# AIflowerQ/InvPref_KDD_2022

Hardware: AMD Instinct MI355X
Metric: training interactions/sec, Yahoo-implicit InvPref (higher is better)
Workload: dtype f32; 1 GPU; yahoo_r3_implicit_shaped; users=15400, items=1000, envs=4, factor_num=64, scaling=strong, interactions_total=250154, global_batch=8192, interactions_per_gpu=250154, batch_per_gpu=8192, estep_every_steps=155, parallelism=single GPU

## Files before the change

invpref_kdd_2022_amd/csrc/canon_math.hpp:

```cpp
#pragma once
#include <hip/hip_runtime.h>

namespace invpref {

__device__ __forceinline__ float bits_to_float(unsigned u) { return __builtin_bit_cast(float, u); }
__device__ __forceinline__ unsigned float_to_bits(float f) { return __builtin_bit_cast(unsigned, f); }

__device__ __forceinline__ float pow2i(int n) { return bits_to_float((unsigned)(n + 127) << 23); }

__device__ __forceinline__ float c_exp(float x) {
    float n = __builtin_rintf(x * 1.44269504f);
    float r = __builtin_fmaf(n, -0.693359375f, x);
    r = __builtin_fmaf(n, 2.12194440e-4f, r);
    float p = 1.9875691500e-4f;
    p = __builtin_fmaf(p, r, 1.3981999507e-3f);
    p = __builtin_fmaf(p, r, 8.3334519073e-3f);
    p = __builtin_fmaf(p, r, 4.1665795894e-2f);
    p = __builtin_fmaf(p, r, 1.6666665459e-1f);
    p = __builtin_fmaf(p, r, 5.0000001201e-1f);
    float r2 = r * r;
    float y = __builtin_fmaf(p, r2, r);
    y = y + 1.0f;
    int ni = (int)n;
    int h = ni >> 1;
// ... 28 lines not shown
    float r = m + y;
    r = __builtin_fmaf(fe, 0.693359375f, r);
    r = (x == __builtin_inff()) ? x : r;
    r = (x == 0.0f) ? -__builtin_inff() : r;
    r = (x < 0.0f) ? __builtin_nanf("") : r;
    r = (x != x) ? x : r;
    return r;
}

__device__ __forceinline__ float c_log1p(float x) {
    float u = 1.0f + x;
    float r = c_log(u) * (x / (u - 1.0f));
    return (u == 1.0f) ? x : r;
}

__device__ __forceinline__ float c_sigmoid(float x) { return 1.0f / (1.0f + c_exp(-x)); }

__device__ __forceinline__ float c_bce(float s, float y) {
    float a = c_log1p(-s);
    a = a > -100.0f ? a : -100.0f;
    float b = c_log(s);
    b = b > -100.0f ? b : -100.0f;
    return (y - 1.0f) * a - y * b;
}

__device__ __forceinline__ float c_bce_binary(float s, float y) {
    const float x = -s, u = 1.0f + x;
    const bool one = y == 1.0f;
    float l = c_log(one ? s : u);
    const float l1p = (u == 1.0f) ? x : l * (x / (u - 1.0f));
    l = one ? l : l1p;
    l = l > -100.0f ? l : -100.0f;
    return -l;
}

__device__ __forceinline__ float c_dbce(float s, float y) {
    float d = (1.0f - s) * s;
    d = d > 1e-12f ? d : 1e-12f;
    return (s - y) / d;
}

__device__ __forceinline__ float c_sign(float x) { return (float)((x > 0.0f) - (x < 0.0f)); }

__device__ __forceinline__ float f_rcp(float x) { return __builtin_amdgcn_rcpf(x); }
__device__ __forceinline__ float f_exp(float x) { return __builtin_amdgcn_exp2f(x * 1.44269504f); }
__device__ __forceinline__ float f_log(float x) { return __builtin_amdgcn_logf(x) * 0.693147181f; }
__device__ __forceinline__ float f_sigmoid(float x) { return f_rcp(1.0f + f_exp(-x)); }
__device__ __forceinline__ float f_bce(float s, float y) {
    float a = f_log(1.0f - s);
    a = a > -100.0f ? a : -100.0f;
    float b = f_log(s);
    b = b > -100.0f ? b : -100.0f;
    return (y - 1.0f) * a - y * b;
}
__device__ __forceinline__ float f_bce_binary(float s, float y) {
    float l = f_log(y == 1.0f ? s : 1.0f - s);
    l = l > -100.0f ? l : -100.0f;
    return -l;
}
__device__ __forceinline__ float f_dbce(float s, float y) {
    float d = (1.0f - s) * s;
    d = d > 1e-12f ? d : 1e-12f;
    return (s - y) * f_rcp(d);
}

template <int CTRL>
__device__ __forceinline__ float dpp_move(float v) {
    return __builtin_bit_cast(float, __builtin_amdgcn_update_dpp(0, __builtin_bit_cast(int, v), CTRL, 0xF, 0xF, true));
}
__device__ __forceinline__ float row16_sum(float x) {
    x = x + dpp_move<0xB1>(x);
    x = x + dpp_move<0x4E>(x);
    x = x + dpp_move<0x141>(x);
    x = x + dpp_move<0x140>(x);
    return x;
}
__device__ __forceinline__ float row16_min(float x) {
    x = __builtin_fminf(x, dpp_move<0xB1>(x));
    x = __builtin_fminf(x, dpp_move<0x4E>(x));
    x = __builtin_fminf(x, dpp_move<0x141>(x));
    x = __builtin_fminf(x, dpp_move<0x140>(x));
    return x;
}
__device__ __forceinline__ float row16_max(float x) {
    x = __builtin_fmaxf(x, dpp_move<0xB1>(x));
    x = __builtin_fmaxf(x, dpp_move<0x4E>(x));
    x = __builtin_fmaxf(x, dpp_move<0x141>(x));
    x = __builtin_fmaxf(x, dpp_move<0x140>(x));
    return x;
}

}
```

invpref_kdd_2022_amd/csrc/invpref_kernels.hip:

```cpp
#include "adam_apply.hpp"
#include "launch.hpp"

using namespace invpref;

namespace {

template <int NC, bool VEC, int EMAX>
__global__ __launch_bounds__(256) void forward_kernel(DevTables t, const int64_t *__restrict__ users,
                                                      const int64_t *__restrict__ items,
                                                      const int64_t *__restrict__ envs, int64_t B, uint32_t flags,
                                                      float *__restrict__ inv, float *__restrict__ envaware,
                                                      float *__restrict__ envout) {
    extern __shared__ __attribute__((aligned(16))) float lds[];
    constexpr int DP = NC * 64;
    float *sEv = lds, *sW = lds + t.E * DP, *sb = sW + t.E * DP;
    stage_table(sEv, t.Ev, t.E, t.D, DP);
    stage_table(sW, t.W, t.E, t.D, DP);
    for (int i = threadIdx.x; i < t.E; i += blockDim.x) sb[i] = t.b[i];
    __syncthreads();
    const int l16 = threadIdx.x & 15;
    const int64_t rows_per_block = blockDim.x / kRow;
    const bool implicit = flags & INVPREF_IMPLICIT;
    for (int64_t s = blockIdx.x * rows_per_block + (threadIdx.x >> 4); s < B; s += gridDim.x * rows_per_block) {
        const int64_t u = users[s], v = items[s];
// ... 422 lines not shown
                                                          int sched_slot) {
    if (sched_state) a = sched_last_launch(sched_state, sched_table, sched_n, sched_slot);
    const int64_t total = r.end4[r.n - 1];
    for (int64_t j = blockIdx.x * (int64_t)blockDim.x + threadIdx.x; j < total; j += (int64_t)gridDim.x * blockDim.x) {
        int q = 0;
        while (j >= r.end4[q]) q++;
        const int64_t i = r.off4[q] + (j - (q ? r.end4[q - 1] : 0));
        adam_f4_at(p, g, m, v, i, a, zero_grad);
    }
}

constexpr int kEpsTableMaxE = 7;
struct EpsBase { float v[INVPREF_MAX_ENVS]; };
struct Factorials { unsigned long long f[INVPREF_MAX_ENVS + 1]; };
__device__ __forceinline__ unsigned long long unrank_packed(unsigned long long r, int E, const Factorials &fac) {
    unsigned avail = (1u << E) - 1u;
    unsigned long long out = 0;
#pragma unroll
    for (int pos = 0; pos < INVPREF_MAX_ENVS; pos++) {
        if (pos < E) {
            unsigned long long f = 1;
#pragma unroll
            for (int k = 0; k < INVPREF_MAX_ENVS; k++) f = (k == E - 1 - pos) ? fac.f[k] : f;
            const unsigned d = (unsigned)(r / f);
            r -= (unsigned long long)d * f;
            unsigned seen = 0, pick = 0;
#pragma unroll
            for (int b = 0; b < INVPREF_MAX_ENVS; b++) {
                const bool on = (avail >> b) & 1u;
                pick = (on && seen == d) ? (unsigned)b : pick;
                seen += on ? 1u : 0u;
            }
            avail &= ~(1u << pick);
            out |= (unsigned long long)pick << (4 * pos);
        }
    }
    return out;
}
__device__ __forceinline__ unsigned unrank_packed_small(unsigned r, int E) {
    unsigned c[8];
    c[0] = 0;
#pragma unroll
    for (int k = 1; k < 8; k++) { c[k] = r % (unsigned)(k + 1); r /= (unsigned)(k + 1); }
    unsigned avail = (1u << E) - 1u, out = 0;
#pragma unroll
    for (int pos = 0; pos < kEpsTableMaxE; pos++) {
        if (pos < E) {
            unsigned d = 0;
#pragma unroll
            for (int k = 0; k < 8; k++) d = (k == E - 1 - pos) ? c[k] : d;
            unsigned seen = 0, pick = 0;
#pragma unroll
            for (int b = 0; b < 8; b++) {
                const bool on = (avail >> b) & 1u;
                pick = (on && seen == d) ? (unsigned)b : pick;
                seen += on ? 1u : 0u;
            }
            avail &= ~(1u << pick);
            out |= pick << (4 * pos);
        }
    }
    return out;
}
template <typename IT>
__global__ __launch_bounds__(256) void eps_unrank_kernel(const IT *__restrict__ idx, int64_t N, int E, Factorials fac,
                                                         unsigned long long *__restrict__ packed) {
    for (int64_t s = blockIdx.x * (int64_t)blockDim.x + threadIdx.x; s < N; s += (int64_t)gridDim.x * blockDim.x)
        packed[s] = unrank_packed(min((unsigned long long)idx[s], fac.f[E] - 1ull), E, fac);
}
constexpr int kTicketShards = 32;
struct EstepFin {
    int *state;
    int64_t *ring;
    int ring_cap;
    int64_t *counts;
    int64_t *diff;
    float *class_w;
    const unsigned *perm_table;
};
__device__ __forceinline__ int ld_sc1_i(const int *p) { return __hip_atomic_load(p, __ATOMIC_RELAXED, __HIP_MEMORY_SCOPE_AGENT); }
__device__ __forceinline__ void st_sc1_i(int *p, int v) { __hip_atomic_store(p, v, __ATOMIC_RELAXED, __HIP_MEMORY_SCOPE_AGENT); }

constexpr int kEstepNumSgpr = 80;
template <int NC, bool VEC, bool NARROW>
__global__ __launch_bounds__(256) __attribute__((amdgpu_num_sgpr(kEstepNumSgpr))) void estep_assign_kernel(DevTables t, const int64_t *__restrict__ users,
                                                           const int64_t *__restrict__ items,
                                                           const float *__restrict__ scores, int64_t N, uint32_t flags,
                                                           const float *__restrict__ eps_rows,
                                                           const unsigned long long *__restrict__ eps_packed, EpsBase eps_base,
                                                           const void *__restrict__ eps_index, int eps_index_bytes,
                                                           int eps_rows_n, Factorials fac,
                                                           const int64_t *old_envs, int64_t *new_envs,
                                                           int *slabs, EstepFin fin) {
    extern __shared__ __attribute__((aligned(16))) float lds[];
    constexpr int DP = NC * 64;
    float *sEv = lds;
    int *cnt = reinterpret_cast<int *>(lds + t.E * DP);
    float *sbase = lds + t.E * DP + INVPREF_MAX_ENVS + 1;
    stage_table(sEv, t.Ev, t.E, t.D, DP);
    for (int i = threadIdx.x; i <= t.E; i += blockDim.x) cnt[i] = 0;
    unsigned *stab = reinterpret_cast<unsigned *>(sbase + INVPREF_MAX_ENVS);
    if (eps_packed || eps_index) {
#pragma unroll
        for (int k = 0; k < INVPREF_MAX_ENVS; k++)
            if (threadIdx.x == k) sbase[k] = eps_base.v[k];
    }
    const int64_t rows_per_block = blockDim.x / kRow;
    const int64_t chunk = ((N + gridDim.x - 1) / gridDim.x + rows_per_block - 1) / rows_per_block * rows_per_block;
    const int64_t s_begin = blockIdx.x * chunk, s_end = min(N, s_begin + chunk);
    auto load_idx = [&](int64_t sx) -> unsigned {
        return eps_index_bytes == 1 ? (unsigned)reinterpret_cast<const uint8_t *>(eps_index)[sx]
                                    : (unsigned)reinterpret_cast<const int32_t *>(eps_index)[sx];
    };
    if (eps_index) {
        if (fin.perm_table)
            for (int i = threadIdx.x; i < eps_rows_n; i += blockDim.x) stab[i] = fin.perm_table[i];
        else
            for (int i = threadIdx.x; i < eps_rows_n; i += blockDim.x) stab[i] = unrank_packed_small((unsigned)i, t.E);
    }
    __syncthreads();
    const int l16 = threadIdx.x & 15;
    const bool implicit = flags & INVPREF_IMPLICIT;
    float eps_thr = 0.f;
    if (eps_packed || eps_index) {
        float mx = 0.f;
#pragma unroll
        for (int k = 0; k < INVPREF_MAX_ENVS; k++) mx = (k < t.E) ? __builtin_fmaxf(mx, __builtin_fabsf(eps_base.v[k])) : mx;
        eps_thr = mx * 67108864.f * 1.001f;
    }
    const int64_t s_first = s_begin + (threadIdx.x >> 4);
    const bool idx_bulk = eps_index && eps_index_bytes == 1;
    const int lane64 = threadIdx.x & 63, grp_w = lane64 >> 4;
    auto load_bulk = [&](int blk) -> unsigned {
        const int64_t sx = s_begin + ((threadIdx.x >> 6) * 4 + (lane64 & 3)) + rows_per_block * ((int64_t)blk * 16 + (lane64 >> 2));
        return sx < s_end ? (unsigned)reinterpret_cast<const uint8_t *>(eps_index)[sx] : 0u;
    };
    unsigned bulk_cur = idx_bulk ? load_bulk(0) : 0u, bulk_next = 0u;
    unsigned idx_cur = (eps_index && !idx_bulk && s_first < s_end) ? load_idx(s_first) : 0u;
    int pass = 0;
    for (int64_t s = s_first; s < s_end; s += rows_per_block, pass++) {
        unsigned idx_next = 0u;
        if (idx_bulk) {
            const int pk = __builtin_amdgcn_readfirstlane(pass);
            if ((pk & 15) == 0) {
                if (pk) bulk_cur = bulk_next;
                bulk_next = load_bulk((pk >> 4) + 1);
            }
            const int src = (pk & 15) * 4;
            const unsigned i0 = __builtin_amdgcn_readlane(bulk_cur, src), i1 = __builtin_amdgcn_readlane(bulk_cur, src + 1);
            const unsigned i2 = __builtin_amdgcn_readlane(bulk_cur, src + 2), i3 = __builtin_amdgcn_readlane(bulk_cur, src + 3);
            idx_cur = grp_w == 0 ? i0 : (grp_w == 1 ? i1 : (grp_w == 2 ? i2 : i3));
        } else if (eps_index && s + rows_per_block < s_end) {
            idx_next = load_idx(s + rows_per_block);
        }
        const int64_t u = users[s], v = items[s];
        const float y = scores[s];
        float4 pu[NC], qi[NC], pa[NC], qa[NC];
        if (NARROW) {
            const unsigned uo = (unsigned)u * (unsigned)t.D, vo = (unsigned)v * (unsigned)t.D;
            load_row<NC, VEC>(t.Pu + uo, 0, t.D, l16, pu);
            load_row<NC, VEC>(t.Qi + vo, 0, t.D, l16, qi);
            load_row<NC, VEC>(t.Pa + uo, 0, t.D, l16, pa);
            load_row<NC, VEC>(t.Qa + vo, 0, t.D, l16, qa);
        } else {
            load_row<NC, VEC>(t.Pu, u, t.D, l16, pu);
            load_row<NC, VEC>(t.Qi, v, t.D, l16, qi);
            load_row<NC, VEC>(t.Pa, u, t.D, l16, pa);
            load_row<NC, VEC>(t.Qa, v, t.D, l16, qa);
        }
        const float p = dot2<NC>(pu, qi);
        const float sp = implicit ? c_sigmoid(p) : p;
        float qmine = 0.f;
        for (int c = 0; c < t.E; c++) {
            float4 ev[NC];
            lds_row<NC>(sEv, c, l16, ev);
            const float q = dot3<NC>(pa, qa, ev);
            qmine = (l16 == c) ? q : qmine;
        }
        float dist;
        if (implicit) {
            const float sv = sp * c_sigmoid(qmine);
            const bool binary = __builtin_amdgcn_ballot_w64(!(y == 0.0f || y == 1.0f)) == 0;
            dist = binary ? c_bce_binary(sv, y) : c_bce(sv, y);
        } else { const float r = (p + qmine) - y; dist = r * r; }
        if (eps_rows && l16 < t.E) dist = dist + eps_rows[s * t.E + l16];
        if (eps_packed || eps_index) {
            const bool need = row16_min(l16 < t.E ? dist : __builtin_inff()) < eps_thr;
            if (need) {
                if (eps_packed && l16 < t.E) dist = dist + sbase[(eps_packed[s] >> (4 * l16)) & 15ull];
                if (eps_index && l16 < t.E)
                    dist = dist + sbase[(stab[min(idx_cur, (unsigned)(eps_rows_n - 1))] >> (4 * l16)) & 15u];
            }
        }
        dist = l16 < t.E ? dist : __builtin_inff();
        const float dmin = row16_min(dist);
        const int bi_num = (int)row16_min(dist == dmin ? (float)l16 : 99.f);
        const int bi_nan = (int)row16_min(dist != dist ? (float)l16 : 99.f);
        const int bi = bi_nan < 99 ? bi_nan : bi_num;
        if (l16 == 0) {
            const int64_t was = old_envs ? old_envs[s] : (int64_t)bi;
            const bool changed = was != (int64_t)bi;
            new_envs[s] = bi;
            atomicAdd(cnt + bi, 1);
            if (changed) atomicAdd(cnt + t.E, 1);
        }
        if (!idx_bulk) idx_cur = idx_next;
    }
    __syncthreads();
    if (!fin.state) {
        for (int i = threadIdx.x; i <= t.E; i += blockDim.x) slabs[(int64_t)blockIdx.x * (t.E + 1) + i] = cnt[i];
        return;
    }
    __shared__ int s_last;
    __shared__ long long s_tot[INVPREF_MAX_ENVS + 1];
    if (threadIdx.x < 64) {
        if ((int)threadIdx.x <= t.E) {
            const int S0 = min(kTicketShards, (int)gridDim.x);
            __hip_atomic_fetch_add(fin.state + 32 + 32 * ((int)blockIdx.x % S0) + 1 + (int)threadIdx.x, cnt[threadIdx.x], __ATOMIC_RELAXED,
                                   __HIP_MEMORY_SCOPE_AGENT);
        }
        asm volatile("s_waitcnt vmcnt(0)" ::: "memory");
        if (threadIdx.x == 0) {
            const int S = min(kTicketShards, (int)gridDim.x), sh = (int)blockIdx.x % S;
            const int members = ((int)gridDim.x - sh + S - 1) / S;
            int *tk = fin.state + 32 + 32 * sh;
            int last = 0;
            if (__hip_atomic_fetch_add(tk, 1, __ATOMIC_RELAXED, __HIP_MEMORY_SCOPE_AGENT) == members - 1) {
                st_sc1_i(tk, 0);
                last = __hip_atomic_fetch_add(fin.state, 1, __ATOMIC_RELAXED, __HIP_MEMORY_SCOPE_AGENT) == S - 1;
            }
            s_last = last;
        }
    }
    for (int i = threadIdx.x; i <= t.E; i += blockDim.x) s_tot[i] = 0;
    __syncthreads();
    if (!s_last) return;
    {
        const int E1 = t.E + 1, nsl = (int)gridDim.x;
        const int S0 = min(kTicketShards, nsl);
        for (int i = threadIdx.x; i < S0 * E1; i += blockDim.x) {
            int *w = fin.state + 32 + 32 * (i / E1) + 1 + i % E1;
            const int x = ld_sc1_i(w);
            st_sc1_i(w, 0);
            atomicAdd((unsigned long long *)&s_tot[i % E1], (unsigned long long)(long long)x);
        }
        __syncthreads();
        int64_t *row = nullptr;
        if (fin.ring) row = fin.ring + (int64_t)((unsigned)fin.state[1] % (unsigned)fin.ring_cap) * E1;
        if ((int)threadIdx.x < t.E) {
            const long long c = s_tot[threadIdx.x];
            const long long r = (c + 1 < N - 1) ? c + 1 : N - 1;
            if (fin.counts) fin.counts[threadIdx.x] = c;
            if (fin.class_w) fin.class_w[threadIdx.x] = (float)((double)r / (double)N);
            if (row) row[threadIdx.x] = c;
        }
        if (threadIdx.x == 0) {
            if (fin.diff) *fin.diff = s_tot[t.E];
            if (row) row[t.E] = s_tot[t.E];
        }
        __syncthreads();
        if (threadIdx.x == 0) {
            if (fin.ring) fin.state[1] = fin.state[1] + 1;
            st_sc1_i(fin.state, 0);
        }
    }
}

__global__ __launch_bounds__(256) void env_hist_kernel(const int64_t *__restrict__ envs, int64_t N, int E,
                                                       int *__restrict__ slabs) {
    __shared__ int cnt[INVPREF_MAX_ENVS + 1];
    for (int i = threadIdx.x; i <= E; i += blockDim.x) cnt[i] = 0;
    __syncthreads();
    for (int64_t s = blockIdx.x * (int64_t)blockDim.x + threadIdx.x; s < N; s += (int64_t)gridDim.x * blockDim.x)
        atomicAdd(cnt + (int)envs[s], 1);
    __syncthreads();
    for (int i = threadIdx.x; i <= E; i += blockDim.x) slabs[(int64_t)blockIdx.x * (E + 1) + i] = cnt[i];
}

__global__ __launch_bounds__(256) void stat_envs_kernel(const int64_t *__restrict__ envs, int64_t N, int E,
                                                        const int *__restrict__ slabs, int nslabs,
                                                        int64_t *__restrict__ counts, int64_t *__restrict__ diff,
                                                        float *__restrict__ class_w, float *__restrict__ sample_w) {
    __shared__ long long tot[INVPREF_MAX_ENVS + 1];
    __shared__ float cw[INVPREF_MAX_ENVS];
    for (int i = threadIdx.x; i <= E; i += blockDim.x) tot[i] = 0;
    __syncthreads();
    long long acc[INVPREF_MAX_ENVS + 1];
#pragma unroll
    for (int c = 0; c <= INVPREF_MAX_ENVS; c++) acc[c] = 0;
// ... 82 lines not shown
#pragma unroll
    for (int c = 0; c < DC; c++)
#pragma unroll
        for (int s = 0; s < 16; s++) a[c][s] = pu[64 * c + 4 * s];
    const int tiles = (I + 15) / 16;
    const int t0 = (int)blockIdx.y * steps_per, t1 = min(tiles, t0 + steps_per);
    if (t0 >= t1) return;
    constexpr int F4 = D / 4, PER = 16 * F4 / 256;
    static_assert(PER == DC, "staging: DC float4 per thread");
    int src_off[PER], dst_off[PER], rr[PER];
#pragma unroll
    for (int j = 0; j < PER; j++) {
        const int f = threadIdx.x + 256 * j;
        rr[j] = f / F4;
        src_off[j] = 4 * (f - rr[j] * F4);
        dst_off[j] = rr[j] * RS + src_off[j];
    }
    float4 st[PER];
#pragma unroll
    for (int j = 0; j < PER; j++)
        st[j] = *reinterpret_cast<const float4 *>(Qi + (int64_t)min(t0 * 16 + rr[j], I - 1) * D + src_off[j]);
#pragma unroll
    for (int j = 0; j < PER; j++) *reinterpret_cast<float4 *>(lds + dst_off[j]) = st[j];
    __syncthreads();
    for (int t = t0; t < t1; t++) {
        const int buf = (t - t0) & 1;
        const int tn = min(t + 1, t1 - 1);
#pragma unroll
        for (int j = 0; j < PER; j++)
            st[j] = *reinterpret_cast<const float4 *>(Qi + (int64_t)min(tn * 16 + rr[j], I - 1) * D + src_off[j]);
        const float *bt = lds + buf * TILE + m * RS + k;
        f32x4_t acc[16];
#pragma unroll
        for (int s = 0; s < 16; s++) acc[s] = f32x4_t{0.f, 0.f, 0.f, 0.f};
#pragma unroll
        for (int c = 0; c < DC; c++)
#pragma unroll
            for (int s = 0; s < 16; s++)
                acc[s] = __builtin_amdgcn_mfma_f32_16x16x4f32(a[c][s], bt[64 * c + 4 * s], acc[s], 0, 0, 0);
#pragma unroll
        for (int s = 0; s < 16; s += 2) acc[s] = acc[s] + acc[s + 1];
#pragma unroll
        for (int s = 0; s < 16; s += 4) acc[s] = acc[s] + acc[s + 2];
#pragma unroll
        for (int s = 0; s < 16; s += 8) acc[s] = acc[s] + acc[s + 4];
        acc[0] = acc[0] + acc[8];
        const int item = t * 16 + m;
#pragma unroll
        for (int r = 0; r < 4; r++) {
            float p = acc[0][r];
            if (apply_sigmoid) p = c_sigmoid(p);
            const int64_t row = (int64_t)blockIdx.x * 64 + wave * 16 + 4 * k + r;
            if (row < n && item < I) out[row * (int64_t)I + item] = p;
        }
#pragma unroll
        for (int j = 0; j < PER; j++) *reinterpret_cast<float4 *>(lds + (buf ^ 1) * TILE + dst_off[j]) = st[j];
        __syncthreads();
    }
}

__global__ __launch_bounds__(256) void sample_weights_kernel(const int64_t *__restrict__ envs, int64_t N_local,
                                                             const int64_t *__restrict__ counts, int64_t N_total, int E,
                                                             float *__restrict__ class_w, float *__restrict__ sample_w) {
    __shared__ float cw[INVPREF_MAX_ENVS];
    if (threadIdx.x < E) {
        const long long c = counts[threadIdx.x];
        const long long r = (c + 1 < N_total - 1) ? c + 1 : N_total - 1;
        const float w = (float)((double)r / (double)N_total);
        cw[threadIdx.x] = w;
        if (blockIdx.x == 0 && class_w) class_w[threadIdx.x] = w;
    }
    __syncthreads();
    if (sample_w)
        for (int64_t s = blockIdx.x * (int64_t)blockDim.x + threadIdx.x; s < N_local; s += (int64_t)gridDim.x * blockDim.x)
            sample_w[s] = cw[(int)envs[s]];
}

constexpr int kMstepThreads = 512, kMstepMaxBlocks = 512;
constexpr int kEstepThreads = 256, kEstepMaxBlocks = 2048;
inline int mstep_blocks(int64_t B) {
    int64_t nb = (B + (kMstepThreads / kRow) - 1) / (kMstepThreads / kRow);
    return (int)(nb < 1 ? 1 : (nb > kMstepMaxBlocks ? kMstepMaxBlocks : nb));
}
inline int estep_blocks(int64_t N) {
    int64_t nb = (N + (kEstepThreads / kRow) - 1) / (kEstepThreads / kRow);
    static const int cap_env = std::getenv("INVPREF_ESTEP_BLOCKS") ? atoi(std::getenv("INVPREF_ESTEP_BLOCKS")) : 0;
    const int cap = cap_env > 0 && cap_env < kEstepMaxBlocks ? cap_env : kEstepMaxBlocks;
    return (int)(nb < 1 ? 1 : (nb > cap ? cap : nb));
}

template <typename F>
int with_nv(int nc, bool vec, F &&f) {
    return with_bool(vec, [&](auto vec_c) {
        return with_int<1, 2, 4>(nc, [&](auto nc_c) {
            if constexpr (!decltype(vec_c)::value && decltype(nc_c)::value != 4) return (int)INVPREF_EUNSUPPORTED;
            else return f(nc_c, vec_c);
        });
    });
}
template <typename F>
int with_nve(int nc, bool vec, int emax, F &&f) {
    return with_nv(nc, vec, [&](auto nc_c, auto vec_c) {
        return with_int<4, 8, 16>(emax, [&](auto emax_c) { return f(nc_c, vec_c, emax_c); });
    });
}

}

template <bool UNPACK, bool VEC>
__global__ __launch_bounds__(256) void pack_rows_kernel(float *__restrict__ flat, const int64_t *__restrict__ row_offsets,
                                                        int64_t n_rows, int32_t D, int64_t tail_offset, int64_t tail_len,
                                                        float *__restrict__ packed) {
    constexpr int W = VEC ? 4 : 1;
    const int64_t per_row = D / W, body = n_rows * per_row, total = body + (tail_len + W - 1) / W;
    for (int64_t i = (int64_t)blockIdx.x * blockDim.x + threadIdx.x; i < total; i += (int64_t)gridDim.x * blockDim.x) {
        float *f, *q;
        int cnt = W;
        if (i < body) {
            const int64_t r = i / per_row, c = i - r * per_row;
            f = flat + row_offsets[r] + c * W;
            q = packed + r * (int64_t)D + c * W;
        } else {
            const int64_t c = (i - body) * W;
            f = flat + tail_offset + c;
            q = packed + n_rows * (int64_t)D + c;
            if (tail_len - c < W) cnt = (int)(tail_len - c);
        }
        if (VEC && cnt == 4) {
            if (UNPACK) *reinterpret_cast<float4 *>(f) = *reinterpret_cast<const float4 *>(q);
            else *reinterpret_cast<float4 *>(q) = *reinterpret_cast<const float4 *>(f);
        } else {
            for (int k = 0; k < cnt; k++) {
                if (UNPACK) f[k] = q[k];
                else q[k] = f[k];
            }
        }
    }
}

static int pack_rows_launch(bool unpack, float *flat, const int64_t *row_offsets, int64_t n_rows, int32_t D,
                            int64_t tail_offset, int64_t tail_len, float *packed, int vec_ok, void *stream) {
    if (!flat || !packed || n_rows < 0 || D < 1 || tail_len < 0 || tail_offset < 0 || (n_rows > 0 && !row_offsets))
        return INVPREF_EINVAL;
    if (n_rows == 0 && tail_len == 0) return 0;
    const uintptr_t af = reinterpret_cast<uintptr_t>(flat), aq = reinterpret_cast<uintptr_t>(packed);
    const bool vec = vec_ok && D % 4 == 0 && tail_offset % 4 == 0 && ((af | aq) & 15u) == 0;
    const int64_t items = n_rows * (D / (vec ? 4 : 1)) + (tail_len + (vec ? 3 : 0)) / (vec ? 4 : 1);
    int64_t nb = (items + 255) / 256;
    nb = nb < 1 ? 1 : (nb > 4096 ? 4096 : nb);
    return with_bool(unpack, [&](auto unpack_c) {
        return with_bool(vec, [&](auto vec_c) {
            hipLaunchKernelGGL((pack_rows_kernel<decltype(unpack_c)::value, decltype(vec_c)::value>), dim3((unsigned)nb), dim3(256),
                               0, (hipStream_t)stream, flat, row_offsets, n_rows, D, tail_offset, tail_len, packed);
            return (int)hipGetLastError();
        });
    });
}

template <bool BACKWARD>
static int launch_mstep_atomic(const InvPrefTables *tables, const InvPrefTables *grads, const int64_t *users,
                               const int64_t *items, const int64_t *envs, const float *scores, const float *sample_weights,
                               int64_t B, const StepScalars &k, uint32_t flags, const Upstream &up, float l2, float l1,
                               int64_t batch_norm, float *losses6, void *workspace, hipStream_t st) {
    const DevTables t = dev_tables(tables);
    const DevGrads g = dev_grads(grads);
    const bool vec = vec_ok(tables) && vec_ok(grads);
    const int nc = vec ? nc_of(t.D) : 4, emax = emax_of(t.E);
    const int DP = nc * 64, EDP = t.E * DP;
// ... 183 lines not shown
         reinterpret_cast<uintptr_t>(exp_avg_sq)) & 15u)
        return INVPREF_EINVAL;
    if (sched && (!sched->state || !sched->table || sched->n <= 0)) return INVPREF_EINVAL;
    AdamRanges r{};
    int64_t total = 0;
    for (int i = 0; i < n_ranges; i++) {
        if (offsets[i] < 0 || lengths[i] <= 0 || (offsets[i] & 3) || (lengths[i] & 3)) return INVPREF_EINVAL;
        r.off4[i] = offsets[i] >> 2;
        total += lengths[i] >> 2;
        r.end4[i] = total;
    }
    r.n = n_ranges;
    int64_t nb = (total + 255) / 256;
    if (nb > 2048) nb = 2048;
    hipLaunchKernelGGL(adam_ranges_kernel, dim3((unsigned)nb), dim3(256), 0, (hipStream_t)stream, param, grad, exp_avg,
                       exp_avg_sq, r, a, zero_grad, sched ? sched->state : nullptr,
                       sched ? reinterpret_cast<const SchedRow *>(sched->table) : nullptr, sched ? sched->n : 0,
                       sched ? (sched->slot & 1) : 0);
    return (int)hipGetLastError();
}

int invpref_adam_ranges_hip(float *param, float *grad, float *exp_avg, float *exp_avg_sq, const int64_t *offsets,
                            const int64_t *lengths, int32_t n_ranges, int64_t step, double lr, double beta1, double beta2,
                            double eps, int zero_grad, void *stream) {
    if (step < 1) return INVPREF_EINVAL;
    return adam_ranges_launch(param, grad, exp_avg, exp_avg_sq, offsets, lengths, n_ranges,
                              adam_scalars(step, lr, beta1, beta2, eps), zero_grad, nullptr, stream);
}

int invpref_adam_ranges_sched_hip(float *param, float *grad, float *exp_avg, float *exp_avg_sq, const int64_t *offsets,
                                  const int64_t *lengths, int32_t n_ranges, const InvPrefAdamSchedule *sched,
                                  int zero_grad, void *stream) {
    if (!sched) return INVPREF_EINVAL;
    return adam_ranges_launch(param, grad, exp_avg, exp_avg_sq, offsets, lengths, n_ranges, AdamScalars{}, zero_grad,
                              sched, stream);
}

size_t invpref_estep_workspace_bytes(const InvPrefTables *tables, int64_t N) {
    const int64_t E = tables ? tables->env_num : INVPREF_MAX_ENVS;
    return sizeof(int) * (size_t)(E + 1) * kEstepMaxBlocks + sizeof(unsigned long long) * (size_t)(N > 0 ? N : 0);
}

int invpref_stat_envs_hip(const int64_t *envs, int64_t N, int64_t env_num, int64_t *counts, float *class_weights,
                          float *sample_weights, void *workspace, size_t workspace_bytes, void *stream) {
    if (!envs || !counts || !workspace || N <= 0 || env_num <= 0) return INVPREF_EINVAL;
    if (env_num > INVPREF_MAX_ENVS) return INVPREF_EUNSUPPORTED;
    if (workspace_bytes < sizeof(int) * (size_t)(env_num + 1) * kEstepMaxBlocks) return INVPREF_EWORKSPACE;
    int64_t nb = (N + 255) / 256;
    if (nb > kEstepMaxBlocks) nb = kEstepMaxBlocks;
    hipStream_t st = (hipStream_t)stream;
    int *slabs = (int *)workspace;
    hipLaunchKernelGGL(env_hist_kernel, dim3((unsigned)nb), dim3(256), 0, st, envs, N, (int)env_num, slabs);
    hipLaunchKernelGGL(stat_envs_kernel, dim3((unsigned)nb), dim3(256), 0, st, envs, N, (int)env_num, slabs, (int)nb,
                       counts, (int64_t *)nullptr, class_weights, sample_weights);
    return (int)hipGetLastError();
}

int invpref_sample_weights_hip(const int64_t *envs, int64_t N_local, const int64_t *counts, int64_t N_total,
                               int64_t env_num, float *class_weights, float *sample_weights, void *stream) {
    if (!counts || N_local < 0 || N_total <= 0 || env_num <= 0 || (N_local > 0 && sample_weights && !envs))
        return INVPREF_EINVAL;
    if (env_num > INVPREF_MAX_ENVS) return INVPREF_EUNSUPPORTED;
    int64_t nb = (N_local + 255) / 256;
    if (nb < 1) nb = 1;
    if (nb > kEstepMaxBlocks) nb = kEstepMaxBlocks;
    hipLaunchKernelGGL(sample_weights_kernel, dim3((unsigned)nb), dim3(256), 0, (hipStream_t)stream, envs, N_local, counts,
                       N_total, (int)env_num, class_weights, sample_weights);
    return (int)hipGetLastError();
}

static int estep_launch(const InvPrefTables *tables, const int64_t *users, const int64_t *items, const float *scores,
                        int64_t N, uint32_t flags, const float *eps_rows, const void *perm_index, int index_bytes,
                        const float *eps_base_host, const int64_t *old_envs, int64_t *new_envs, int64_t *counts,
                        int64_t *diff, float *class_weights, float *sample_weights, void *workspace,
                        size_t workspace_bytes, void *stream, const EstepFin *fused = nullptr) {
    int rc = check_tables(tables);
    if (rc) return rc;
    if (N <= 0 || !users || !items || !scores || !new_envs || !workspace) return INVPREF_EINVAL;
    if (!fused && (!counts || !diff)) return INVPREF_EINVAL;
    if (workspace_bytes < invpref_estep_workspace_bytes(tables, N)) return INVPREF_EWORKSPACE;
    const DevTables t = dev_tables(tables);
    const bool vec = vec_ok(tables);
    const int nc = vec ? nc_of(t.D) : 4;
    const int nb = estep_blocks(N);
    const size_t lds = sizeof(float) * ((size_t)t.E * nc * 64 + INVPREF_MAX_ENVS + 1 + INVPREF_MAX_ENVS);
    hipStream_t st = (hipStream_t)stream;
    int *slabs = (int *)workspace;
    unsigned long long *eps_packed = nullptr;
    EpsBase eps_base{};
    Factorials fac{};
    fac.f[0] = 1;
    for (int k = 1; k <= INVPREF_MAX_ENVS; k++) fac.f[k] = fac.f[k - 1] * (unsigned long long)k;
    const void *eps_index = nullptr;
    int eps_rows_n = 0;
    size_t lds_extra = 0;
    if (perm_index) {
        if (eps_rows || !eps_base_host || (index_bytes != 1 && index_bytes != 4 && index_bytes != 8)) return INVPREF_EINVAL;
        if ((index_bytes == 1 && t.E > 5) || (index_bytes == 4 && t.E > 12)) return INVPREF_EINVAL;
        for (int k = 0; k < t.E; k++) eps_base.v[k] = eps_base_host[k];
    }
    bool table_form = perm_index && t.E <= kEpsTableMaxE && index_bytes != 8;
    if (table_form) {
        lds_extra = sizeof(unsigned) * (size_t)fac.f[t.E];
        if (lds + lds_extra > 64 * 1024) { table_form = false; lds_extra = 0; }
    }
    if (table_form) {
        eps_index = perm_index;
        eps_rows_n = (int)fac.f[t.E];
    } else if (perm_index) {
        eps_packed = reinterpret_cast<unsigned long long *>(reinterpret_cast<char *>(workspace) +
                                                           sizeof(int) * (size_t)(t.E + 1) * kEstepMaxBlocks);
        int64_t ub = (N + 255) / 256;
        if (ub > 4096) ub = 4096;
        with_int<1, 4, 8>(index_bytes, [&](auto bytes_c) {
            constexpr int W = decltype(bytes_c)::value;
            using IT = std::conditional_t<W == 1, uint8_t, std::conditional_t<W == 4, int32_t, int64_t>>;
            hipLaunchKernelGGL(eps_unrank_kernel<IT>, dim3((unsigned)ub), dim3(256), 0, st, (const IT *)perm_index, N, t.E, fac,
                               eps_packed);
            return 0;
        });
    }
    EstepFin fin{};
    if (fused) {
        fin = *fused;
        if (!table_form) fin.perm_table = nullptr;
    }
    static const bool force64 = std::getenv("INVPREF_ESTEP_OFFSETS64") != nullptr && std::getenv("INVPREF_ESTEP_OFFSETS64")[0] == '1';
    const bool narrow = !force64 && (uint64_t)std::max(t.U, t.I) * (uint64_t)t.D * 4u < (1ull << 32);
    rc = with_nv(nc, vec, [&](auto nc_c, auto vec_c) {
        return with_bool(narrow, [&](auto narrow_c) {
            hipLaunchKernelGGL((estep_assign_kernel<decltype(nc_c)::value, decltype(vec_c)::value, decltype(narrow_c)::value>),
                               dim3(nb), dim3(kEstepThreads), lds + lds_extra, st, t, users, items, scores, N, flags, eps_rows,
                               eps_packed, eps_base, eps_index, index_bytes, eps_rows_n, fac, old_envs, new_envs, slabs, fin);
            return (int)hipGetLastError();
        });
    });
    if (rc) return rc;
    if (fused) return 0;
    int64_t nb2 = (N + 255) / 256;
    if (nb2 > 256) nb2 = 256;
    hipLaunchKernelGGL(stat_envs_kernel, dim3((unsigned)nb2), dim3(256), 0, st, new_envs, N, t.E, slabs, nb, counts, diff,
                       class_weights, sample_weights);
    return (int)hipGetLastError();
}

int invpref_estep_hip(const InvPrefTables *tables, const int64_t *users, const int64_t *items, const float *scores,
                      int64_t N, uint32_t flags, const float *eps_rows, const int64_t *old_envs, int64_t *new_envs,
                      int64_t *counts, int64_t *diff, float *class_weights, float *sample_weights, void *workspace,
                      size_t workspace_bytes, void *stream) {
    return estep_launch(tables, users, items, scores, N, flags, eps_rows, nullptr, 0, nullptr, old_envs, new_envs, counts,
                        diff, class_weights, sample_weights, workspace, workspace_bytes, stream);
}

int invpref_estep_perm_hip(const InvPrefTables *tables, const int64_t *users, const int64_t *items, const float *scores,
                           int64_t N, uint32_t flags, const void *perm_index, int index_bytes, const float *eps_base,
                           const int64_t *old_envs, int64_t *new_envs, int64_t *counts, int64_t *diff,
                           float *class_weights, float *sample_weights, void *workspace, size_t workspace_bytes,
                           void *stream) {
    if (!perm_index) return INVPREF_EINVAL;
    return estep_launch(tables, users, items, scores, N, flags, nullptr, perm_index, index_bytes, eps_base, old_envs,
                        new_envs, counts, diff, class_weights, sample_weights, workspace, workspace_bytes, stream);
}

int invpref_perm_table_fill(int32_t env_num, uint32_t *host_table) {
    if (!host_table || env_num < 1 || env_num > kEpsTableMaxE) return INVPREF_EINVAL;
    int rows = 1;
    for (int k = 2; k <= env_num; k++) rows *= k;
    for (int r = 0; r < rows; r++) {
        unsigned avail = (1u << env_num) - 1u, out = 0;
        int rem = r, f = rows;
        for (int pos = 0; pos < env_num; pos++) {
            f /= (env_num - pos);
            const int d = rem / f;
            rem -= d * f;
            int seen = 0, pick = 0;
            for (int b = 0; b < env_num; b++)
                if ((avail >> b) & 1u) { if (seen == d) pick = b; seen++; }
            avail &= ~(1u << pick);
            out |= (unsigned)pick << (4 * pos);
        }
        host_table[r] = out;
    }
    return rows;
}

int invpref_estep_fused_hip(const InvPrefTables *tables, const int64_t *users, const int64_t *items, const float *scores,
                            int64_t N, uint32_t flags, const void *perm_index, int index_bytes, const float *eps_base,
                            const uint32_t *perm_table, int64_t *envs, int32_t *state, int64_t *ring, int32_t ring_cap,
                            int64_t *counts, int64_t *diff, float *class_weights, void *workspace, size_t workspace_bytes,
                            void *stream) {
    if (!state || !envs || (ring && ring_cap <= 0)) return INVPREF_EINVAL;
    EstepFin fin{};
    fin.state = state; fin.ring = ring; fin.ring_cap = ring_cap; fin.counts = counts; fin.diff = diff;
    fin.class_w = class_weights; fin.perm_table = perm_table;
    return estep_launch(tables, users, items, scores, N, flags, nullptr, perm_index, perm_index ? index_bytes : 0, eps_base, envs,
                        envs, counts, diff, class_weights, nullptr, workspace, workspace_bytes, stream, &fin);
}

}
```

Before: 533.6 million interactions/s.

## Pack four samples per 16-lane group in E-step assign with DPP env lanes

Adds a packed E-step variant for D<=64 and E<=4. Each 16-lane row group processes four samples, fetching IDs through DPP quad broadcasts. Each lane of a quad then owns one environment's distance, with argmin done by quad DPP reductions. This cuts the rows-per-pass redundancy and per-sample overhead, launches more rows per block, and requests high occupancy via waves_per_eu. It adds branching complexity and register pressure and only runs when the shape constraints hold.

```diff
diff --git a/invpref_kdd_2022_amd/csrc/canon_math.hpp b/invpref_kdd_2022_amd/csrc/canon_math.hpp
--- a/invpref_kdd_2022_amd/csrc/canon_math.hpp
+++ b/invpref_kdd_2022_amd/csrc/canon_math.hpp
@@ -134,6 +134,20 @@
     x = __builtin_fminf(x, dpp_move<0x140>(x));
     return x;
 }
+__device__ __forceinline__ float quad_min(float x) {
+    x = __builtin_fminf(x, dpp_move<0xB1>(x));
+    x = __builtin_fminf(x, dpp_move<0x4E>(x));
+    return x;
+}
+template <int J>
+__device__ __forceinline__ unsigned quad_bcast(unsigned v) {
+    return (unsigned)__builtin_amdgcn_update_dpp(0, (int)v, J * 0x55, 0xF, 0xF, true);
+}
+template <int J>
+__device__ __forceinline__ float quad_keep(float old, float v) {
+    return __builtin_bit_cast(float, __builtin_amdgcn_update_dpp(__builtin_bit_cast(int, old), __builtin_bit_cast(int, v), 0xE4, 0xF,
+                                                                 1 << J, false));
+}
 __device__ __forceinline__ float row16_max(float x) {
     x = __builtin_fmaxf(x, dpp_move<0xB1>(x));
     x = __builtin_fmaxf(x, dpp_move<0x4E>(x));
diff --git a/invpref_kdd_2022_amd/csrc/invpref_kernels.hip b/invpref_kdd_2022_amd/csrc/invpref_kernels.hip
--- a/invpref_kdd_2022_amd/csrc/invpref_kernels.hip
+++ b/invpref_kdd_2022_amd/csrc/invpref_kernels.hip
@@ -528,8 +528,9 @@
 __device__ __forceinline__ void st_sc1_i(int *p, int v) { __hip_atomic_store(p, v, __ATOMIC_RELAXED, __HIP_MEMORY_SCOPE_AGENT); }
 
 constexpr int kEstepNumSgpr = 80;
-template <int NC, bool VEC, bool NARROW>
-__global__ __launch_bounds__(256) __attribute__((amdgpu_num_sgpr(kEstepNumSgpr))) void estep_assign_kernel(DevTables t, const int64_t *__restrict__ users,
+constexpr int kEstepPackedMaxE = 4;
+template <int NC, bool VEC, bool NARROW, bool PACKED>
+__global__ __launch_bounds__(256) __attribute__((amdgpu_num_sgpr(kEstepNumSgpr), amdgpu_waves_per_eu(PACKED ? 8 : 1))) void estep_assign_kernel(DevTables t, const int64_t *__restrict__ users,
                                                            const int64_t *__restrict__ items,
                                                            const float *__restrict__ scores, int64_t N, uint32_t flags,
                                                            const float *__restrict__ eps_rows,
@@ -551,7 +552,7 @@
         for (int k = 0; k < INVPREF_MAX_ENVS; k++)
             if (threadIdx.x == k) sbase[k] = eps_base.v[k];
     }
-    const int64_t rows_per_block = blockDim.x / kRow;
+    const int64_t rows_per_block = PACKED ? blockDim.x / 4 : blockDim.x / kRow;
     const int64_t chunk = ((N + gridDim.x - 1) / gridDim.x + rows_per_block - 1) / rows_per_block * rows_per_block;
     const int64_t s_begin = blockIdx.x * chunk, s_end = min(N, s_begin + chunk);
     auto load_idx = [&](int64_t sx) -> unsigned {
@@ -574,6 +575,129 @@
         for (int k = 0; k < INVPREF_MAX_ENVS; k++) mx = (k < t.E) ? __builtin_fmaxf(mx, __builtin_fabsf(eps_base.v[k])) : mx;
         eps_thr = mx * 67108864.f * 1.001f;
     }
+    if constexpr (PACKED) {
+        static_assert(NC == 1 && VEC, "the packed loop is written for one float4 chunk per lane");
+        const int wave = __builtin_amdgcn_readfirstlane((int)(threadIdx.x >> 6));
+        const unsigned lane64 = threadIdx.x & 63u, e4 = l16 & 3;
+        const unsigned off_g = (lane64 >> 4) * 4 + e4, off_c = lane64 >> 2;
+        const unsigned off_b = (lane64 >> 4) * (unsigned)rows_per_block + (lane64 & 15u);
+        const bool row_on = l16 * 4 < t.D;
+        const unsigned lane_byte = row_on ? (unsigned)l16 * 16u : 0u;
+        const unsigned row_bytes = (unsigned)t.D * 4u;
+        const int64_t w_first = s_begin + wave * 16;
+        auto room = [&](int64_t base, int cap) -> unsigned {
+            const int64_t r = s_end - 1 - base;
+            return (unsigned)__builtin_amdgcn_readfirstlane((int)(r < cap ? r : cap));
+        };
+        auto at = [](auto *arr, int64_t base, unsigned byte_off) -> auto & {
+            using T = std::remove_pointer_t<decltype(arr)>;
+            using C = std::conditional_t<std::is_const_v<T>, const char, char>;
+            auto *p = arr + base;
+            asm("" : "+s"(p));
+            return *reinterpret_cast<T *>(reinterpret_cast<C *>(p) + byte_off);
+        };
+        const bool idx_bulk = eps_index && eps_index_bytes == 1;
+        auto load_bulk = [&](int64_t base) -> unsigned {
+            const unsigned lim = room(base, 255);
+            return off_b <= lim ? (unsigned)at(reinterpret_cast<const uint8_t *>(eps_index), base, off_b) : 0u;
+        };
+        auto load_ids = [&](int64_t base, unsigned &ur, unsigned &vr, float &y, unsigned &idx) {
+            const unsigned lim = room(base, 15), og = min(off_g, lim), oc = min(off_c, lim);
+            const int64_t u = at(users, base, og * 8u), v = at(items, base, og * 8u);
+            if constexpr (NARROW) { ur = (unsigned)u * row_bytes; vr = (unsigned)v * row_bytes; }
+            else { ur = (unsigned)u; vr = (unsigned)v; }
+            const float yy = at(scores, base, oc * 4u);
+            y = off_c <= lim ? yy : 0.f;
+            if (eps_index && !idx_bulk) idx = (unsigned)at(reinterpret_cast<const int32_t *>(eps_index), base, oc * 4u);
+        };
+        auto row = [&](const float *tab, unsigned r) -> float4 {
+            const char *b = reinterpret_cast<const char *>(tab);
+            if constexpr (NARROW) return *reinterpret_cast<const float4 *>(b + (r + lane_byte));
+            else {
+                uint64_t off = (uint64_t)r * row_bytes + lane_byte;
+                asm("" : "+v"(off));
+                return *reinterpret_cast<const float4 *>(b + off);
+            }
+        };
+        unsigned ur_n = 0, vr_n = 0;
+        float y_n = 0.f;
+        unsigned idx_n = 0u, bulk_cur = 0u, bulk_next = 0u;
+        if (w_first < s_end) {
+            load_ids(w_first, ur_n, vr_n, y_n, idx_n);
+            if (idx_bulk) bulk_next = load_bulk(w_first);
+        }
+        int pass = 0;
+        for (int64_t base = w_first; base < s_end; base += rows_per_block, pass++) {
+            const unsigned ur = ur_n, vr = vr_n;
+            const float y = y_n;
+            unsigned idx_cur = idx_n;
+            const unsigned lim = room(base, 15);
+            if (base + rows_per_block < s_end) load_ids(base + rows_per_block, ur_n, vr_n, y_n, idx_n);
+            if (idx_bulk) {
+                if ((pass & 3) == 0) {
+                    bulk_cur = bulk_next;
+                    bulk_next = base + 4 * rows_per_block < s_end ? load_bulk(base + 4 * rows_per_block) : 0u;
+                }
+                idx_cur = (unsigned)__builtin_amdgcn_ds_bpermute((int)(((pass & 3) * 16 + off_c) * 4), (int)bulk_cur);
+            }
+            float pq = 0.f, qc[kEstepPackedMaxE] = {0.f, 0.f, 0.f, 0.f};
+            auto inner = [&](auto jc) {
+                constexpr int J = decltype(jc)::value;
+                const unsigned uj = quad_bcast<J>(ur), vj = quad_bcast<J>(vr);
+                const float4 pu = row(t.Pu, uj), qi = row(t.Qi, vj), pa = row(t.Pa, uj), qa = row(t.Qa, vj);
+                float sp = 0.f;
+                sp = __builtin_fmaf(pu.x, qi.x, sp); sp = __builtin_fmaf(pu.y, qi.y, sp);
+                sp = __builtin_fmaf(pu.z, qi.z, sp); sp = __builtin_fmaf(pu.w, qi.w, sp);
+                pq = quad_keep<J>(pq, row16_sum(row_on ? sp : 0.f));
+                const float4 ab = f4mul(pa, qa);
+#pragma unroll
+                for (int c = 0; c < kEstepPackedMaxE; c++) {
+                    float4 ev[1];
+                    lds_row<1>(sEv, min(c, t.E - 1), l16, ev);
+                    float sq = 0.f;
+                    sq = __builtin_fmaf(ab.x, ev[0].x, sq); sq = __builtin_fmaf(ab.y, ev[0].y, sq);
+                    sq = __builtin_fmaf(ab.z, ev[0].z, sq); sq = __builtin_fmaf(ab.w, ev[0].w, sq);
+                    qc[c] = quad_keep<J>(qc[c], row16_sum(row_on ? sq : 0.f));
+                }
+            };
+            inner(std::integral_constant<int, 0>{});
+            asm volatile("" ::: "memory");
+            inner(std::integral_constant<int, 1>{});
+            asm volatile("" ::: "memory");
+            inner(std::integral_constant<int, 2>{});
+            asm volatile("" ::: "memory");
+            inner(std::integral_constant<int, 3>{});
+            asm volatile("" ::: "memory");
+            const float qmine = e4 == 0 ? qc[0] : (e4 == 1 ? qc[1] : (e4 == 2 ? qc[2] : qc[3]));
+            const bool live = off_c <= lim, lane_on = live && (int)e4 < t.E;
+            float dist;
+            if (implicit) {
+                const float sv = c_sigmoid(pq) * c_sigmoid(qmine);
+                const bool binary = __builtin_amdgcn_ballot_w64(!(y == 0.0f || y == 1.0f)) == 0;
+                dist = binary ? c_bce_binary(sv, y) : c_bce(sv, y);
+            } else { const float r = (pq + qmine) - y; dist = r * r; }
+            if (eps_rows && lane_on) dist = dist + at(eps_rows, base * t.E, (off_c * (unsigned)t.E + e4) * 4u);
+            if (eps_packed || eps_index) {
+                const bool need = quad_min(lane_on ? dist : __builtin_inff()) < eps_thr;
+                if (need && lane_on) {
+                    if (eps_packed) dist = dist + sbase[(at(eps_packed, base, off_c * 8u) >> (4 * e4)) & 15ull];
+                    if (eps_index) dist = dist + sbase[(stab[min(idx_cur, (unsigned)(eps_rows_n - 1))] >> (4 * e4)) & 15u];
+                }
+            }
+            dist = lane_on ? dist : __builtin_inff();
+            const float dmin = quad_min(dist);
+            const int bi_num = (int)quad_min(dist == dmin ? (float)e4 : 99.f);
+            const int bi_nan = (int)quad_min(dist != dist ? (float)e4 : 99.f);
+            const int bi = bi_nan < 99 ? bi_nan : bi_num;
+            if (e4 == 0 && live) {
+                const int64_t was = old_envs ? at(old_envs, base, off_c * 8u) : (int64_t)bi;
+                const bool changed = was != (int64_t)bi;
+                at(new_envs, base, off_c * 8u) = bi;
+                atomicAdd(cnt + bi, 1);
+                if (changed) atomicAdd(cnt + t.E, 1);
+            }
+        }
+    } else {
     const int64_t s_first = s_begin + (threadIdx.x >> 4);
     const bool idx_bulk = eps_index && eps_index_bytes == 1;
     const int lane64 = threadIdx.x & 63, grp_w = lane64 >> 4;
@@ -651,6 +775,7 @@
             if (changed) atomicAdd(cnt + t.E, 1);
         }
         if (!idx_bulk) idx_cur = idx_next;
+    }
     }
     __syncthreads();
     if (!fin.state) {
@@ -899,8 +1024,8 @@
     int64_t nb = (B + (kMstepThreads / kRow) - 1) / (kMstepThreads / kRow);
     return (int)(nb < 1 ? 1 : (nb > kMstepMaxBlocks ? kMstepMaxBlocks : nb));
 }
-inline int estep_blocks(int64_t N) {
-    int64_t nb = (N + (kEstepThreads / kRow) - 1) / (kEstepThreads / kRow);
+inline int estep_blocks(int64_t N, int per_pass = kEstepThreads / kRow) {
+    int64_t nb = (N + per_pass - 1) / per_pass;
     static const int cap_env = std::getenv("INVPREF_ESTEP_BLOCKS") ? atoi(std::getenv("INVPREF_ESTEP_BLOCKS")) : 0;
     const int cap = cap_env > 0 && cap_env < kEstepMaxBlocks ? cap_env : kEstepMaxBlocks;
     return (int)(nb < 1 ? 1 : (nb > cap ? cap : nb));
@@ -1250,7 +1375,8 @@
     const DevTables t = dev_tables(tables);
     const bool vec = vec_ok(tables);
     const int nc = vec ? nc_of(t.D) : 4;
-    const int nb = estep_blocks(N);
+    const bool packed = nc == 1 && t.E <= kEstepPackedMaxE;
+    const int nb = packed ? estep_blocks(N, kEstepThreads / 4) : estep_blocks(N);
     const size_t lds = sizeof(float) * ((size_t)t.E * nc * 64 + INVPREF_MAX_ENVS + 1 + INVPREF_MAX_ENVS);
     hipStream_t st = (hipStream_t)stream;
     int *slabs = (int *)workspace;
@@ -1297,10 +1423,16 @@
     const bool narrow = !force64 && (uint64_t)std::max(t.U, t.I) * (uint64_t)t.D * 4u < (1ull << 32);
     rc = with_nv(nc, vec, [&](auto nc_c, auto vec_c) {
         return with_bool(narrow, [&](auto narrow_c) {
-            hipLaunchKernelGGL((estep_assign_kernel<decltype(nc_c)::value, decltype(vec_c)::value, decltype(narrow_c)::value>),
-                               dim3(nb), dim3(kEstepThreads), lds + lds_extra, st, t, users, items, scores, N, flags, eps_rows,
-                               eps_packed, eps_base, eps_index, index_bytes, eps_rows_n, fac, old_envs, new_envs, slabs, fin);
-            return (int)hipGetLastError();
+            return with_bool(packed, [&](auto packed_c) {
+                constexpr int NC = decltype(nc_c)::value;
+                if constexpr (decltype(packed_c)::value && NC != 1) return (int)INVPREF_EUNSUPPORTED;
+                else {
+                    hipLaunchKernelGGL((estep_assign_kernel<NC, decltype(vec_c)::value, decltype(narrow_c)::value, decltype(packed_c)::value>),
+                                       dim3(nb), dim3(kEstepThreads), lds + lds_extra, st, t, users, items, scores, N, flags, eps_rows,
+                                       eps_packed, eps_base, eps_index, index_bytes, eps_rows_n, fac, old_envs, new_envs, slabs, fin);
+                    return (int)hipGetLastError();
+                }
+            });
         });
     });
     if (rc) return rc;
```

Measured after the change: 535.3 million interactions/s, median of 3. Within noise of the previous version (+0.3%).
